# CederGroupHub/sparse-lm

Hardware: AMD Instinct MI355X
Metric: fits/sec over 50-alpha Lasso path at n=100k p=5k (higher is better)
Workload: dtype f64

## Files before the change

sparse-lm_amd/csrc/host_logic.hpp:

```cpp
#pragma once
#include <stddef.h>
#include <math.h>
#include <stdint.h>
#include <stdio.h>
#include <stdlib.h>

#include <algorithm>
#include <utility>
#include <vector>

#if defined(__HIPCC__)
#define SLM_HD __host__ __device__
#else
#define SLM_HD
#endif

namespace slm_host {

struct PoolLedger {
  struct Idle { int dev; size_t bytes; void* block; };
  struct Live { void* block; int dev; size_t bytes; };
  std::vector<Idle> idle;
  std::vector<Live> live;
  size_t idle_bytes = 0;

  void* take(int dev, size_t bytes) {
    for (size_t i = 0; i < idle.size(); ++i) {
      if (idle[i].dev == dev && idle[i].bytes == bytes) {
        void* p = idle[i].block;
        idle.erase(idle.begin() + (long)i);
        idle_bytes -= bytes;
        live.push_back({p, dev, bytes});
        return p;
      }
    }
    return nullptr;
  }
  void adopt(void* p, int dev, size_t bytes) { live.push_back({p, dev, bytes}); }

  bool give_back(void* p, size_t cap, bool pooling, std::vector<void*>* evict) {
    for (size_t i = 0; i < live.size(); ++i) {
      if (live[i].block != p) continue;
      const int dev = live[i].dev;
      const size_t bytes = live[i].bytes;
      live.erase(live.begin() + (long)i);
      if (!pooling || bytes > cap) return false;
      while (idle_bytes + bytes > cap && !idle.empty()) {
        evict->push_back(idle.front().block);
        idle_bytes -= idle.front().bytes;
        idle.erase(idle.begin());
      }
      idle.push_back({dev, bytes, p});
      idle_bytes += bytes;
      return true;
    }
    return false;
  }
  std::vector<void*> retire_device(int dev) {
    std::vector<void*> out;
    for (const Live& e : live)
      if (e.dev == dev) return out;
    for (size_t i = 0; i < idle.size();) {
      if (idle[i].dev == dev) {
        out.push_back(idle[i].block);
        idle_bytes -= idle[i].bytes;
        idle.erase(idle.begin() + (long)i);
      } else {
        ++i;
      }
    }
    return out;
  }
  std::vector<void*> flush() {
    std::vector<void*> out;
    for (const Idle& e : idle) out.push_back(e.block);
    idle.clear();
    idle_bytes = 0;
    return out;
  }
};

inline int row_sets(int n_lanes, const void* const* row_weight, const int64_t* n_eff, int* set_of, int* set_lane) {
  int n_sets = 0;
  for (int l = 0; l < n_lanes; ++l) {
    int found = -1;
    for (int m = 0; m < l && found < 0; ++m)
      if (row_weight[m] == row_weight[l] && n_eff[m] == n_eff[l]) found = set_of[m];
    if (found < 0) {
      found = n_sets;
      set_lane[n_sets++] = l;
    }
    set_of[l] = found;
  }
  return n_sets;
}

struct LaneWalk {
  int32_t first;
  int32_t n_points;
  int32_t stride;
  int32_t tail_pt;
};
inline LaneWalk interleaved_walk(int lane, int B, int64_t total, bool tail_band, bool slack_deep = false) {
  LaneWalk w;
  w.first = lane;
  w.n_points = (int32_t)total;
  w.stride = B;
  w.tail_pt = -1;
  const int64_t rem = total % B, n_reg = total - rem;
  if (slack_deep && tail_band && total > 2 * (int64_t)B && total <= 3 * (int64_t)B) {
    const int64_t e = (3 * (int64_t)B - total) / 2, F = B - e;
    if (e >= 1 && F >= 1) {
      if (lane >= F) {
        w.n_points = (int32_t)B;
      } else {
        w.n_points = (int32_t)(B + F);
        const int64_t t = B + F + lane;
        if (t < total) w.tail_pt = (int32_t)t;
      }
      return w;
    }
  }
  if (tail_band && rem > 0 && n_reg >= 2 * (int64_t)B) {
    w.n_points = (int32_t)n_reg;
    if (lane >= B - rem) w.tail_pt = (int32_t)(n_reg + (lane - (B - rem)));
  }
  return w;
}
inline int64_t interleaved_points(const LaneWalk& w) {
  const int64_t regular = w.n_points > w.first ? ((int64_t)w.n_points - w.first + w.stride - 1) / w.stride : 0;
  return regular + (w.tail_pt >= 0 ? 1 : 0);
}

struct XtrGrid { int xb, yb, rows; };
inline int auto_path_lanes(int64_t n_points, int cap, bool big, bool wide_ok) {
  if (n_points < 1) n_points = 1;
  const int narrow = (int)std::min<int64_t>(std::min(cap, 16), n_points);
  if (!big || cap < 20 || n_points <= 16) return narrow;
  int best = narrow;
  double best_cost = 1.45 * (double)((n_points + 15) / 16);
  auto offer = [&](int64_t lanes) {
    lanes = std::min(lanes, n_points);
    if (lanes <= 16 || lanes > cap) return;
    const int64_t passes = (n_points + lanes - 1) / lanes;
    const double cost = (double)passes * ((lanes <= 20 ? 1.03 : 1.22) + 0.45);
    if (cost < best_cost - 1e-9) {
      best_cost = cost;
      best = (int)lanes;
    }
  };
  offer(18);
  offer(20);
  if (wide_ok)
    for (int64_t passes = 1; passes <= (n_points + 20) / 21; ++passes) {
      const int64_t lanes = (n_points + passes - 1) / passes;
      if (lanes > 20 && lanes <= 32) offer(lanes);
    }
  return best;
}

inline int xtr_row_blocks_most(int cus, int64_t ld, int col_block) {
  const int xb = (int)((ld + col_block - 1) / col_block);
  return std::max(1, 2 * cus / xb);
}
inline XtrGrid xtr_grid(int64_t n, int64_t ld, int col_block, int64_t want) {
  XtrGrid g;
  g.xb = (int)((ld + col_block - 1) / col_block);
  if (want < 1) want = 1;
  int64_t rows = (n + want - 1) / want;
  rows = (rows + 7) / 8 * 8;
  g.rows = (int)rows;
  g.yb = (int)((n + rows - 1) / rows);
  return g;
}

constexpr int kSampleThreads = 256;
constexpr int kSampleWgsPerCu = 4;
constexpr int kSampleMinRows = 16;
struct SamplePlan {
  int xb, yb;
  int64_t rows;
  int64_t ld32;
};
inline int64_t sample_ld32(int64_t p) { return (p + 3) / 4 * 4; }
inline SamplePlan sample_plan(int64_t n_s, int64_t p, int64_t ld32, int cus) {
  SamplePlan g;
  g.ld32 = ld32;
  (void)p;
  const int64_t quads = ld32 / 4;
  g.xb = (int)std::max<int64_t>(1, (quads + kSampleThreads - 1) / kSampleThreads);
  if (n_s < 1) n_s = 1;
  const int64_t want = std::max<int64_t>(1, (int64_t)kSampleWgsPerCu * std::max(1, cus) / g.xb);
  g.rows = std::max<int64_t>(kSampleMinRows, (n_s + want - 1) / want);
  g.yb = (int)((n_s + g.rows - 1) / g.rows);
  return g;
}

template <typename Entry>
inline int find_by_fingerprint(const std::vector<Entry>& entries, double fp1, double fp2, double n_eff) {
  for (size_t i = 0; i < entries.size(); ++i)
    if (entries[i].fp1 == fp1 && entries[i].fp2 == fp2 && entries[i].n_eff == n_eff) return (int)i;
  return -1;
}

inline void triangle_tile(int t, int* I_out, int* J_out) {
  int I = 0;
  while ((I + 1) * (I + 2) / 2 <= t) ++I;
  *I_out = I;
  *J_out = t - I * (I + 1) / 2;
}
inline int triangle_tiles(int side) { return side * (side + 1) / 2; }
SLM_HD inline void triangle_tile_fast(int t, int* I_out, int* J_out) {
  int I = (int)((sqrtf(8.0f * (float)t + 1.0f) - 1.0f) * 0.5f);
  while (I * (I + 1) / 2 > t) --I;
  while ((I + 1) * (I + 2) / 2 <= t) ++I;
  *I_out = I;
  *J_out = t - I * (I + 1) / 2;
}

inline int model_gram_cap(int64_t ld, double budget_bytes, int most) {
  const double each = 4.0 * (double)ld * (double)ld;
  return (int)std::max<double>(1.0, std::min<double>((double)most, budget_bytes / each));
}

constexpr int kSketchPowerIters = 1;
constexpr int kSketchRowDiv = 32;
constexpr int kWsLookahead = 2;
constexpr int kWsPowerIters = 10;

struct Knobs {
  bool split = true;
  double xtr_wgs_per_cu = 1.0;
  int grad_ring = -1;
  int grad_cfg[3] = {0, 0, 0};
  int rowdot_ring = -1;
  bool resid_vec = false;
  int cov_tile = 0;
  int power_iters = 0;
  int ws = -1;
  bool on_chip = true;
  int auto_lanes = 0;
  bool interleave = true;
  bool tail_band = true;
  bool carry = true;
  bool ws_carry = true;
  bool eval_fused = false;
  double ws_theta = 0.85;
  int ws_append = 48;
  int ws_kinit = 0;
  int ws_bb = 1;
  int ws_one_solver = 0;
  bool hard_callwide = false;
  int ws_miss_factor = 4;
  int ws_miss_div = 8;
  double ws_fill = 0.0;
  bool sample_start = true;
  int64_t sample_min_rows = 65536;
  int sample_div = 4;
  bool sample_f64 = false;
  int mg = -1;
  bool handover = true;
  bool light_pass = true;
  bool lag_handover = true;
  bool gram_owner = true;
  double device_pool_gb = -1.0;
  bool allow_any_arch = false;
  int trace = 0;
  bool trace_poll = false;

  template <typename Get>
  static Knobs from(Get get) {
    Knobs k;
    auto text = [&](const char* name) -> const char* { return get(name); };
    auto is_set = [&](const char* name) { return text(name) != nullptr; };
    auto first = [&](const char* name) -> char { const char* e = text(name); return e ? e[0] : '\0'; };
    auto as_int = [&](const char* name, int lo, int hi, int* out) {
      if (const char* e = text(name)) *out = std::max(lo, std::min(hi, atoi(e)));
    };
    k.split = first("SLM_SPLIT") != '0';
    if (const char* e = text("SLM_XTR_WGS_PER_CU")) {
      const double f = atof(e);
      if (f > 0.0 && f <= 2.0) k.xtr_wgs_per_cu = f;
    }
    if (const char c = first("SLM_GRAD_RING")) k.grad_ring = c == '0' ? 0 : (c == '1' ? 1 : -1);
    if (const char* e = text("SLM_GRAD_CONFIG")) {
      int W = 0, C = 0, R = 0;
      if (sscanf(e, "%d,%d,%d", &W, &C, &R) == 3) { k.grad_cfg[0] = W; k.grad_cfg[1] = C; k.grad_cfg[2] = R; }
    }
    if (const char c = first("SLM_ROWDOT_RING")) k.rowdot_ring = c == '1' ? 1 : 0;
    k.resid_vec = first("SLM_RESID_VEC") == '1';
    if (const char* e = text("SLM_COV_TILE")) k.cov_tile = atoi(e);
    if (const char* e = text("SLM_POWER_ITERS")) k.power_iters = std::max(2, atoi(e));
    if (const char c = first("SLM_WS")) k.ws = c == '0' ? 0 : (c == '1' ? 1 : -1);
    k.on_chip = first("SLM_ON_CHIP") != '0';
    if (const char* e = text("SLM_AUTO_LANES")) k.auto_lanes = std::max(1, atoi(e));
    k.interleave = !is_set("SLM_NO_INTERLEAVE");
    k.tail_band = !is_set("SLM_NO_TAIL_BAND");
    k.carry = !is_set("SLM_NO_CARRY");
    k.ws_carry = !is_set("SLM_NO_WS_CARRY");
    k.eval_fused = is_set("SLM_EVAL_FUSED");
    if (const char* e = text("SLM_WS_THETA")) {
      const double v = atof(e);
      if (v > 0.0 && v <= 1.0) k.ws_theta = v;
    }
    as_int("SLM_WS_APPEND", 1, 512, &k.ws_append);
    as_int("SLM_WS_KINIT", 16, 512, &k.ws_kinit);
    if (const char* e = text("SLM_WS_BB")) k.ws_bb = atoi(e) != 0;
    if (const char* e = text("SLM_WS_ONE_SOLVER")) k.ws_one_solver = atoi(e) != 0;
    k.hard_callwide = is_set("SLM_HARD_CALLWIDE");
    as_int("SLM_WS_MISS_FACTOR", 1, 8, &k.ws_miss_factor);
    as_int("SLM_WS_MISS_DIV", 1, 4096, &k.ws_miss_div);
    if (const char* e = text("SLM_WS_FILL")) k.ws_fill = std::max(0.1, std::min(1.0, atof(e)));
    k.sample_start = !is_set("SLM_NO_SAMPLE_START");
    if (const char* e = text("SLM_SAMPLE_START_MIN_ROWS")) k.sample_min_rows = std::max<int64_t>(64, atoll(e));
    as_int("SLM_SAMPLE_DIV", 1, 64, &k.sample_div);
    k.sample_f64 = first("SLM_SAMPLE_F64") == '1';
    if (const char c = first("SLM_MG")) k.mg = c == '0' ? 0 : (c == '2' ? 2 : -1);
    k.handover = !is_set("SLM_NO_HANDOVER");
    k.light_pass = !is_set("SLM_NO_LIGHT_PASS");
    k.gram_owner = !is_set("SLM_NO_GRAM_OWNER");
    k.lag_handover = !is_set("SLM_NO_LAG_HANDOVER");
    if (const char* e = text("SLM_DEVICE_POOL_GB")) k.device_pool_gb = std::max(0.0, atof(e));
    k.allow_any_arch = is_set("SLM_ALLOW_ANY_ARCH");
    if (const char c = first("SLM_TRACE")) k.trace = (c >= '1' && c <= '3') ? c - '0' : 1;
    k.trace_poll = is_set("SLM_TRACE_POLL");
    return k;
  }
};

}
```

sparse-lm_amd/csrc/ws_kernels.hpp:

```cpp
#pragma once
#include <type_traits>
#include <hip/hip_runtime.h>
#include <stdint.h>

#include "tail_kernels.hpp"
#include "newton_kernels.hpp"

namespace slm {

constexpr int WS_KCAP = 512;
constexpr int WS_KLDS = 112;
constexpr int WS_TILES = WS_KCAP / 16;
constexpr int WS_THREADS = 1024;
constexpr int WS_INNER_MAX = 400;
constexpr int WS_BB_ITERS = 14;
constexpr double WS_BB_MAX_STEP = 20.0;
constexpr double WS_INNER_TOL = 0.05;
constexpr int WS_MAX_REPEATS = 6;
constexpr int WS_NEWTON_AFTER = 16;
constexpr int WS_NEWTON_MAX = 256;
constexpr int WS_AFTER_DIRECT = 40;
constexpr double WS_NEWTON_RQ = 0.05;
constexpr int WS_NEWTON_REFUSALS = 4;
constexpr double WS_NEWTON_ENTER = 0.3;
constexpr int WS_NEWTON_RESOLVE = 5;
static_assert(NT_MAXT * NT_B == WS_KCAP, "the direct solve covers a full working set");

struct WsCtl {
  int32_t request;
  int32_t building;
  int32_t valid;
  int32_t K;
  int32_t Kreal;
  int32_t k_new;
  int32_t builds;
  int32_t appends;
  int32_t max_builds;
  int32_t disabled;
  int32_t misses;
  int32_t refined;
  int32_t counter;
  int32_t stale;
  int32_t overflows;
  int32_t sweep_new;
  int32_t sweep_miss;
  int32_t staged;
  int32_t inner_iters;
  int32_t hard;
  int32_t hard_next;
  int32_t newton_steps;
  int32_t newton_fails;
  int32_t newton_nopd;
  int32_t newton_trial[4];
  int32_t newton_ref[4];
  int32_t newton_factors;
  int32_t newton_unknowns;
  unsigned long long nt_ticks[SLM_MAX_LANES][6];
  int32_t nt_factors[SLM_MAX_LANES];
  unsigned long long solve_ticks[5];
  int32_t want_full[SLM_MAX_LANES];
  int32_t iters_hist[32];
  unsigned long long lane_ticks[SLM_MAX_LANES];
  int32_t last_point[SLM_MAX_LANES];
  int32_t repeats[SLM_MAX_LANES];
  int32_t last_cols[SLM_MAX_LANES];
  double Lw[SLM_MAX_LANES];
  int32_t carried;
  int32_t outgrown;
  int32_t served[SLM_MAX_LANES];
  int32_t hard_lane[SLM_MAX_LANES];
};

struct WsArgs {
  WsCtl* ws;
  int32_t* idx;
  int32_t* pos;
  int32_t* gs;
  int32_t* gl;
  double* score;
  double* XW;
  double* part;
  double* Gm;
  double* nt;
  double* Gx;
  const double* X;
  const double* XT;
  int64_t n, ld;
  const double* rw;
  int64_t rw_stride;
  double inv_n[SLM_MAX_LANES];
  int32_t set_of[SLM_MAX_LANES];
  int32_t set_lane[SLM_MAX_LANES];
  int32_t n_sets;
  int32_t nblk;
  const int32_t* owner;
  double theta;
  int32_t lookahead;
  int32_t append_max;
  int32_t k_init;
  int32_t bb_steps;
  int32_t one_solver;
  int32_t miss_factor;
  int32_t miss_div;
  double fill;
  int32_t power_iters;
  int32_t hard_call;
  int32_t keep_full;
};

constexpr int WS_HEAD_WORDS = 24;
static_assert(offsetof(WsCtl, hard_next) / 4 < WS_HEAD_WORDS, "the words the pass kernels decide on");
#define WS_HEAD(hd, field) ((hd)[offsetof(WsCtl, field) / 4])
__device__ __forceinline__ void ws_head_load(const WsCtl* ws, const int* gdone, int32_t* hd) {
  const int tid = threadIdx.x;
  if (tid < WS_HEAD_WORDS) hd[tid] = reinterpret_cast<const int32_t*>(ws)[tid];
  else if (tid == WS_HEAD_WORDS) hd[tid] = gdone ? gdone[0] : 0;
}

static __global__ void ws_ctl_init_kernel(WsCtl* ws, int max_builds) {
  if (threadIdx.x == 0) {
    ws->request = 1;
    ws->max_builds = max_builds;
  }
  if (threadIdx.x < SLM_MAX_LANES) ws->last_point[threadIdx.x] = -1;
}

struct BeginArgs {
  const PathCtl* h_ctl;
  PathCtl* ctl;
  const slm_path_point* h_pts;
  slm_path_point* pts;
  int64_t n_pts;
  int32_t* head;
  int32_t head_words;
  const double* lambda;
  double margin;
  double factor[SLM_MAX_LANES];
  WsCtl* ws;
  int32_t max_builds;
  int32_t n_lanes;
};
static __global__ __launch_bounds__(256) void solve_begin_kernel(SetupArgs s, BeginArgs b) {
  solve_setup_body(s);
  const int64_t stride = (int64_t)gridDim.x * blockDim.x;
  {
    static_assert(sizeof(slm_path_point) == 4 * sizeof(double), "points travel as doubles");
    const double* src = reinterpret_cast<const double*>(b.h_pts);
    double* dst = reinterpret_cast<double*>(b.pts);
    for (int64_t e = (int64_t)blockIdx.x * blockDim.x + threadIdx.x; e < 4 * b.n_pts; e += stride) dst[e] = src[e];
  }
  if (blockIdx.x != 0) return;
  for (int e = threadIdx.x; e < b.head_words; e += 256) b.head[e] = 0;
  {
    static_assert(sizeof(PathCtl) % sizeof(int32_t) == 0, "control blocks travel as words");
    const int32_t* src = reinterpret_cast<const int32_t*>(b.h_ctl);
    int32_t* dst = reinterpret_cast<int32_t*>(b.ctl);
    const int words = b.n_lanes * (int)(sizeof(PathCtl) / sizeof(int32_t));
    for (int e = threadIdx.x; e < words; e += 256) dst[e] = src[e];
  }
  __syncthreads();
  if (b.lambda != nullptr && (int)threadIdx.x < b.n_lanes && threadIdx.x < SLM_MAX_LANES) {
    const int l = threadIdx.x;
    double L0 = b.lambda[0] * b.margin;
    if (L0 <= 0.0) L0 = 1.0;
    const double L = L0 * b.factor[l];
    b.ctl[l].L = L;
    b.ctl[l].ak = 1.25 * L;
    b.ctl[l].Lhat = 0.5 * L0;
  }
  if (b.ws != nullptr) {
    if (threadIdx.x == 0) {
      b.ws->request = 1;
      b.ws->max_builds = b.max_builds;
    }
    if (threadIdx.x < SLM_MAX_LANES) b.ws->last_point[threadIdx.x] = -1;
  }
}

static __global__ __launch_bounds__(256) void ws_ctl_carry_kernel(WsCtl* ws, int max_builds) {
  __shared__ int keep_i[2];
  __shared__ double keep_L[SLM_MAX_LANES];
  if (threadIdx.x == 0) {
    keep_i[0] = ws->K;
    keep_i[1] = ws->Kreal;
  }
  if (threadIdx.x < SLM_MAX_LANES) keep_L[threadIdx.x] = ws->Lw[threadIdx.x];
  __syncthreads();
  int32_t* words = reinterpret_cast<int32_t*>(ws);
  for (int e = threadIdx.x; e < (int)(sizeof(WsCtl) / sizeof(int32_t)); e += 256) words[e] = 0;
  __syncthreads();
  if (threadIdx.x == 0) {
    ws->K = keep_i[0];
    ws->Kreal = keep_i[1];
    ws->valid = 1;
    ws->carried = 1;
    ws->max_builds = max_builds;
  }
  if (threadIdx.x < SLM_MAX_LANES) {
    ws->Lw[threadIdx.x] = keep_L[threadIdx.x];
    ws->last_point[threadIdx.x] = -1;
  }
}

__device__ __forceinline__ int block_excl_scan(int v, int* wave_tot , int* total) {
  const int lane = threadIdx.x & 63, wave = threadIdx.x >> 6;
  int inc = v;
#pragma unroll
  for (int off = 1; off < 64; off <<= 1) {
    const int t = __shfl_up(inc, off, 64);
    if (lane >= off) inc += t;
  }
  __syncthreads();
  if (lane == 63) wave_tot[wave] = inc;
  __syncthreads();
  int base = 0, tot = 0;
#pragma unroll
  for (int w = 0; w < TAIL_WAVES; ++w) {
    const int t = wave_tot[w];
    if (w < wave) base += t;
    tot += t;
  }
  *total = tot;
  return base + inc - v;
}

__device__ __forceinline__ void ws_score_body(TailArgs a, WsArgs w, const int chunk) {
  WsCtl* ws = w.ws;
  const int tid = threadIdx.x;
  __shared__ int32_t hd[WS_HEAD_WORDS + 1];
  __shared__ int lane_np[SLM_MAX_LANES];
  ws_head_load(ws, a.gdone, hd);
  if (tid < SLM_MAX_LANES) lane_np[tid] = tid < a.n_lanes ? a.ctl[tid].n_points : 0;
  __syncthreads();
  if (hd[WS_HEAD_WORDS] != 0 || WS_HEAD(hd, disabled)) return;
  const bool had_w = WS_HEAD(hd, valid) != 0;
  if (!WS_HEAD(hd, request) && !had_w) return;
  if (WS_HEAD(hd, builds) >= WS_HEAD(hd, max_builds) || WS_HEAD(hd, appends) >= 8 * WS_HEAD(hd, max_builds)) return;
  const bool singleton = a.singleton != 0;
  const int nitems = singleton ? a.p : a.G;
  __shared__ int lane_live[SLM_MAX_LANES];
  __shared__ double lane_sa[SLM_MAX_LANES], lane_sb[SLM_MAX_LANES];
  __shared__ int cnt[2];
  if (tid < SLM_MAX_LANES) {
    int live = 0;
    double sa = 0.0, sb = 0.0;
    if (tid < a.n_lanes) {
      const PathCtl* c = a.ctl + tid;
      live = !(c->done || c->idle);
      int path_end = 0;
      for (int l = 0; l < SLM_MAX_LANES; ++l) path_end = max(path_end, lane_np[l]);
      const int end = a.steal ? path_end : c->pt_off + c->n_points;
      int look = min(c->pt_off + c->point + max(w.lookahead, c->stride), end - 1);
      if (c->tail_pt >= 0 && c->point + c->stride >= c->n_points) look = c->pt_off + c->tail_pt;
      const slm_path_point pe = a.pts[look < 0 ? 0 : look];
      sa = pe.sa;
      sb = pe.sb;
    }
    lane_live[tid] = live;
    lane_sa[tid] = sa;
    lane_sb[tid] = sb;
  }
  if (tid == 0) cnt[0] = cnt[1] = 0;
  __syncthreads();

  const double inf = __builtin_huge_val();
  int n_new = 0, n_miss = 0;
  const int gt = chunk * (int)blockDim.x + tid;
  const int it = singleton ? gt : gt >> 4;
  if (singleton) {
    if (it < nitems) {
      double sc = 0.0;
      const int j = it;
      const bool in_w = had_w && w.pos[j] >= 0;
      for (int l0 = 0; l0 < a.n_lanes; l0 += 16) {
        double zp[16], zz[16], aa[16], bb[16], gg[16];
#pragma unroll
        for (int l = 0; l < 16; ++l) {
          const int ll = l0 + l < a.n_lanes ? l0 + l : 0;
          const int64_t off = (int64_t)ll * a.ld;
          zp[l] = a.zprev[off + j];
          zz[l] = a.z[off + j];
          aa[l] = a.a0[off + j];
          bb[l] = a.b0[off + j];
          gg[l] = a.g[(int64_t)ll * (a.ld + 16) + j];
        }
#pragma unroll
        for (int l = 0; l < 16; ++l) {
          if (l0 + l >= a.n_lanes || !lane_live[l0 + l]) continue;
          if (!in_w && had_w && zz[l] != zp[l]) n_miss += 1;
          if (zp[l] != 0.0) {
            sc = inf;
          } else {
            const double thr = lane_sa[l0 + l] * aa[l] + lane_sb[l0 + l] * bb[l];
            sc = fmax(sc, thr > 0.0 ? fabs(gg[l]) / thr : inf);
          }
        }
      }
      if (sc >= w.theta && !in_w) n_new += 1;
      w.score[it] = sc;
    }
  } else {
    static_assert(SLM_MAX_LANES % 16 == 0, "16-thread teams: a thread per (group, lane of a half)");
    const int l16 = tid & 15;
    const bool have = it < nitems;
    double sc = 0.0;
    bool in_w = false;
    int k0 = 0, k1 = 0;
    if (have) {
      k0 = a.gstart[it];
      k1 = a.gstart[it + 1];
      in_w = had_w && w.pos[a.order[k0]] >= 0;
    }
    for (int l = l16; have && l < a.n_lanes; l += 16) {
      if (lane_live[l]) {
        const int64_t off = (int64_t)l * a.ld;
        const double* g = a.g + (int64_t)l * (a.ld + 16);
        double num = 0.0, rmax = 0.0;
        bool act = false;
        for (int k = k0; k < k1; ++k) {
          const int j = a.order[k];
          const double zp = a.zprev[off + j], zj = a.z[off + j], aj = a.a0[off + j], gj = g[j];
          if (!in_w && had_w && zj != zp) n_miss += 1;
          act = act || zp != 0.0;
          const double thr = lane_sa[l] * aj;
          const double m = fmax(fabs(gj) - thr, 0.0);
          num = __builtin_fma(m, m, num);
          rmax = fmax(rmax, thr > 0.0 ? fabs(gj) / thr : inf);
        }
        const double den = lane_sb[l] * a.b0[off + it];
        const double r = den > 0.0 ? sqrt(num) / den : rmax;
        sc = fmax(sc, act ? inf : r);
      }
    }
#pragma unroll
    for (int o = 8; o >= 1; o >>= 1) sc = fmax(sc, __shfl_xor(sc, o, 64));
    if (have && l16 == 0) {
      if (sc >= w.theta && !in_w) n_new += k1 - k0;
      w.score[it] = sc;
    }
  }
  if (n_new) atomicAdd(&cnt[0], n_new);
  if (n_miss) atomicAdd(&cnt[1], n_miss);
  __syncthreads();
  if (tid == 0) {
    if (cnt[0]) atomicAdd(&ws->sweep_new, cnt[0]);
    if (cnt[1]) atomicAdd(&ws->sweep_miss, cnt[1]);
  }
}

static __global__ __launch_bounds__(256) void ws_score_kernel(TailArgs a, WsArgs w) { ws_score_body(a, w, (int)blockIdx.x); }

__device__ __forceinline__ void ws_select_body(TailArgs a, WsArgs w) {
  __shared__ double red[2][TAIL_WAVES];
  __shared__ int wave_tot[TAIL_WAVES];
  WsCtl* ws = w.ws;
  if (threadIdx.x < SLM_MAX_LANES) ws->served[threadIdx.x] = 0;
  if (a.gdone[0] != 0 || ws->disabled) return;
  const int tid = threadIdx.x;
  const int p = a.p, G = a.G;
  const bool singleton = a.singleton != 0;
  const int nitems = singleton ? p : G;
  const bool had_w = ws->valid != 0;

  if (tid == 0 && ws->hard_next) ws->hard = 1;
  const bool requested = ws->request != 0;
  if (!requested && !had_w) return;
  if (ws->builds >= ws->max_builds || ws->appends >= 8 * ws->max_builds) {
    if (tid == 0) {
      ws->request = 0;
      ws->stale = 1;
    }
    return;
  }

  double sweep[2] = {(double)ws->sweep_new, (double)ws->sweep_miss};
  const bool carried = ws->carried != 0;
  __syncthreads();
  if (tid == 0) {
    ws->sweep_new = 0;
    ws->sweep_miss = 0;
    ws->carried = 0;
  }
  const double inf = __builtin_huge_val();
  const bool miss = had_w && sweep[1] != 0.0;
  if (miss && tid == 0) ws->misses += 1;
  if (had_w && !requested && sweep[0] == 0.0) {
    if (miss && tid == 0) ws->stale = 1;
    return;
  }

  const int per = (nitems + WS_THREADS - 1) / WS_THREADS;
  const int i0 = tid * per, i1 = min(i0 + per, nitems);
  const bool cached = per <= 8;
  double c_sc[8];
  int c_sz[8];
  bool c_inw[8];
  if (cached) {
    int first[8];
#pragma unroll
    for (int u = 0; u < 8; ++u) {
      const int it = (i0 + u < i1) ? i0 + u : 0;
      c_sc[u] = (i0 + u < i1) ? w.score[it] : -1.0;
      first[u] = singleton ? it : a.gstart[it];
      c_sz[u] = singleton ? 1 : a.gstart[it + 1] - first[u];
    }
    if (!singleton) {
#pragma unroll
      for (int u = 0; u < 8; ++u) first[u] = a.order[first[u]];
    }
#pragma unroll
    for (int u = 0; u < 8; ++u) c_inw[u] = w.pos[first[u]] >= 0;
  }

  auto count_at = [&](double thr, bool only_new, double* n_sel, double* smax) {
    double v[2] = {0.0, 0.0};
    if (cached) {
#pragma unroll
      for (int u = 0; u < 8; ++u) {
        if (c_sc[u] >= thr && !(only_new && c_inw[u])) v[0] += (double)c_sz[u];
        if (c_sc[u] < inf) v[1] = fmax(v[1], c_sc[u]);
      }
    } else {
      for (int it = tid; it < nitems; it += WS_THREADS) {
        const double sc = w.score[it];
        const int first = singleton ? it : a.order[a.gstart[it]];
        const int size = singleton ? 1 : a.gstart[it + 1] - a.gstart[it];
        if (sc >= thr && !(only_new && w.pos[first] >= 0)) v[0] += (double)size;
        if (sc < inf) v[1] = fmax(v[1], sc);
      }
    }
    double s[1] = {v[0]};
    block_sum<1>(s, red);
    *n_sel = s[0];
    if (smax == nullptr) return;
    double m = v[1];
#pragma unroll
    for (int off = 32; off >= 1; off >>= 1) m = fmax(m, __shfl_xor(m, off, 64));
    __syncthreads();
    if ((tid & 63) == 0) red[1][tid >> 6] = m;
    __syncthreads();
    double mm = 0.0;
#pragma unroll
    for (int k = 0; k < TAIL_WAVES; ++k) mm = fmax(mm, red[1][k]);
    *smax = mm;
  };

  auto fit_threshold = [&](double thr0, bool only_new, double cap, double* n_out) -> double {
    double n_sel, smax;
    count_at(thr0, only_new, &n_sel, &smax);
    if (n_sel <= cap) {
      *n_out = n_sel;
      return thr0;
    }
    double lo = thr0, hi = fmax(smax, thr0) * (1.0 + 1e-12) + 1e-300;
    double n_hi = 0.0;
    for (int k = 0; k < 14; ++k) {
      const double mid = 0.5 * (lo + hi);
      count_at(mid, only_new, &n_sel, nullptr);
      if (n_sel > cap) {
        lo = mid;
      } else {
        hi = mid;
        n_hi = n_sel;
        if (n_sel >= w.fill * cap) break;
      }
    }
    if (n_hi == 0.0) count_at(hi, only_new, &n_hi, nullptr);
    *n_out = n_hi;
    return hi;
  };

  double n_sel, smax, thr = w.theta;
  const int k_old = had_w ? ws->Kreal : 0;
  bool append = had_w;
  if (append) {
    const int miss_mult = miss ? min(w.miss_factor, 1 + (int)sweep[1] / max(w.miss_div, 1)) : 1;
    const double cap = (double)(carried ? max(w.k_init, 4 * w.append_max) : miss_mult * w.append_max);
    if (sweep[0] <= cap) {
      n_sel = sweep[0];
    } else {
      thr = fit_threshold(w.theta, true, cap, &n_sel);
    }
    if (n_sel == 0.0) {
      if (tid == 0) ws->request = 0;
      return;
    }
    if ((double)k_old + n_sel > (double)WS_KCAP) {
      if (tid == 0) ws->outgrown += 1;
      if (w.keep_full) {
        double nz_now;
        count_at(inf, false, &nz_now, nullptr);
        if (nz_now > 0.75 * (double)WS_KCAP) {
          if (tid == 0) {
            ws->request = 0;
            ws->stale = 1;
          }
          return;
        }
      }
      append = false;
      thr = w.theta;
    }
  }
  if (!append) {
    count_at(inf, false, &n_sel, nullptr);
    if (n_sel > (double)WS_KCAP) {
      if (tid == 0) {
        ws->overflows += 1;
        ws->outgrown += 1;
        if (had_w) {
          ws->request = 0;
          ws->stale = 1;
        } else {
          ws->request = 1;
          ws->valid = 0;
          if (ws->overflows >= 50) ws->disabled = 1;
        }
      }
      return;
    }
    const double nonzeros = n_sel;
    thr = fit_threshold(w.theta, false, fmax((double)w.k_init, nonzeros), &n_sel);
    for (int j = tid; j < p; j += WS_THREADS) w.pos[j] = -1;
  }
  for (int k = k_old * (append ? 1 : 0) + tid; k < WS_KCAP; k += WS_THREADS) {
    w.idx[k] = -1;
    w.gs[k] = k;
    w.gl[k] = 1;
  }
  __syncthreads();

  unsigned long long pick = 0ull;
  int mine = 0;
  if (cached) {
#pragma unroll
    for (int u = 0; u < 8; ++u) {
      if (c_sc[u] >= thr && !(append && c_inw[u])) {
        pick |= 1ull << u;
        mine += c_sz[u];
      }
    }
  } else {
    for (int it = i0; it < i1 && it - i0 < 64; ++it) {
      if (!(w.score[it] >= thr)) continue;
      if (append && w.pos[singleton ? it : a.order[a.gstart[it]]] >= 0) continue;
      pick |= 1ull << (it - i0);
      mine += singleton ? 1 : a.gstart[it + 1] - a.gstart[it];
    }
  }
  int total = 0;
  int at = (append ? k_old : 0) + block_excl_scan(mine, wave_tot, &total);
  __syncthreads();
  for (int it = i0; it < i1 && it - i0 < 64; ++it) {
    if (!((pick >> (it - i0)) & 1ull)) continue;
    if (singleton) {
      w.idx[at] = it;
      w.pos[it] = at;
      at += 1;
    } else {
      const int k0 = a.gstart[it], len = a.gstart[it + 1] - k0;
      for (int m = 0; m < len; ++m) {
        const int j = a.order[k0 + m];
        w.idx[at + m] = j;
        w.pos[j] = at + m;
        w.gs[at + m] = at;
        w.gl[at + m] = len;
      }
      at += len;
    }
  }
  if (tid == 0) {
    const int Kreal = (append ? k_old : 0) + total;
    ws->Kreal = Kreal;
    ws->K = max(16, (Kreal + 15) & ~15);
    ws->k_new = append ? k_old : 0;
    ws->building = 1;
    ws->valid = 0;
    ws->stale = 0;
    ws->counter = 0;
    if (append) {
      ws->appends += 1;
    } else {
      ws->builds += 1;
      for (int l = 0; l < SLM_MAX_LANES; ++l) ws->Lw[l] = 0.0;
    }
  }
}

static __global__ __launch_bounds__(WS_THREADS) void ws_select_kernel(TailArgs a, WsArgs w) { ws_select_body(a, w); }

static __global__ __launch_bounds__(256) void ws_gather_kernel(WsArgs w) {
  if (!w.ws->building) return;
  const int K = w.ws->K;
  const int k0 = w.ws->k_new + 32 * (int)blockIdx.y;
  if (k0 >= K) return;
  __shared__ double tile[32][33];
  const int tx = threadIdx.x & 31, ty = threadIdx.x >> 5;
  const int64_t row_tiles = (w.n + 31) / 32;
  int jcol[4];
#pragma unroll
  for (int u = 0; u < 4; ++u) {
    const int k = k0 + ty + 8 * u;
    jcol[u] = k < K ? w.idx[k] : -1;
  }
  for (int64_t rt = blockIdx.x; rt < row_tiles; rt += gridDim.x) {
    const int64_t i0 = rt * 32;
    const int64_t i = i0 + tx;
    double v[4];
#pragma unroll
    for (int u = 0; u < 4; ++u) {
      const int j = jcol[u];
      v[u] = (j >= 0 && i < w.n) ? (w.XT ? w.XT[((rt * w.ld + j) << 5) + tx] : w.X[i * w.ld + j]) : 0.0;
    }
    __syncthreads();
#pragma unroll
    for (int u = 0; u < 4; ++u) tile[ty + 8 * u][tx] = v[u];
    __syncthreads();
    for (int ii = ty; ii < 32; ii += 8) {
      const int64_t i = i0 + ii;
      const int k = k0 + tx;
      if (i < w.n && k < K) w.XW[i * WS_KCAP + k] = tile[tx][ii];
    }
  }
}

struct XtyArgs {
  const WsCtl* ws;
  const int32_t* idx;
  const double* XW;
  const double* y;
  double* part;
  double* g;
  double* gprev;
  double* z;
  PathCtl* ctl;
  const int* done;
  int64_t n, ld;
  double inv_n;
  int n_lanes, nblk;
};
static __global__ __launch_bounds__(512) void ws_xty_partial_kernel(XtyArgs a) {
  if (*a.done) return;
  __shared__ double red[8][WS_KCAP];
  __shared__ double red_yy[8];
  const int K = a.ws->K;
  const int lane = threadIdx.x & 63, wave = threadIdx.x >> 6;
  const int64_t rows = (a.n + gridDim.x - 1) / gridDim.x;
  const int64_t i0 = (int64_t)blockIdx.x * rows, i1 = i0 + rows < a.n ? i0 + rows : a.n;
  double acc[WS_KCAP / 64];
#pragma unroll
  for (int c = 0; c < WS_KCAP / 64; ++c) acc[c] = 0.0;
  double yy = 0.0;
  auto rows4 = [&](auto NC) {
    constexpr int C = decltype(NC)::value;
    for (int64_t i = i0 + wave; i < i1; i += 32) {
      double xv[4][C], yv[4];
#pragma unroll
      for (int r = 0; r < 4; ++r) {
        const bool in = i + 8 * r < i1;
        const int64_t ii = in ? i + 8 * r : i;
        yv[r] = in ? a.y[ii] : 0.0;
#pragma unroll
        for (int c = 0; c < C; ++c) {
          const int k = lane + 64 * c;
          xv[r][c] = a.XW[ii * WS_KCAP + (k < K ? k : 64 * c)];
        }
      }
#pragma unroll
      for (int r = 0; r < 4; ++r) {
        yy = __builtin_fma(yv[r], yv[r], yy);
#pragma unroll
        for (int c = 0; c < C; ++c) acc[c] = __builtin_fma(lane + 64 * c < K ? xv[r][c] : 0.0, yv[r], acc[c]);
      }
    }
  };
  switch ((K + 63) >> 6) {
    case 1: rows4(std::integral_constant<int, 1>{}); break;
    case 2: rows4(std::integral_constant<int, 2>{}); break;
    case 3: rows4(std::integral_constant<int, 3>{}); break;
    case 4: rows4(std::integral_constant<int, 4>{}); break;
    case 5: rows4(std::integral_constant<int, 5>{}); break;
    case 6: rows4(std::integral_constant<int, 6>{}); break;
    case 7: rows4(std::integral_constant<int, 7>{}); break;
    default: rows4(std::integral_constant<int, 8>{}); break;
  }
  static_assert(WS_KCAP / 64 == 8, "eight chunks of 64 positions");
#pragma unroll
  for (int c = 0; c < WS_KCAP / 64; ++c) red[wave][lane + 64 * c] = acc[c];
  if (lane == 0) red_yy[wave] = yy;
  __syncthreads();
  double* out = a.part + (int64_t)blockIdx.x * (WS_KCAP + 1);
  const int k = threadIdx.x;
  if (k < K) {
    double sum = 0.0;
#pragma unroll
    for (int w = 0; w < 8; ++w) sum += red[w][k];
    out[k] = sum;
  }
  if (k == WS_KCAP - 1) {
    double sum = 0.0;
#pragma unroll
    for (int w = 0; w < 8; ++w) sum += red_yy[w];
    out[WS_KCAP] = sum;
  }
}
static __global__ __launch_bounds__(512) void ws_xty_apply_kernel(XtyArgs a) {
  if (*a.done) return;
  __shared__ double red[4][128];
  __shared__ double ry[512];
  const int K = a.ws->K;
  const int kl = threadIdx.x & 127, q = threadIdx.x >> 7;
  const int k = (int)blockIdx.x * 128 + kl;
  if ((int)blockIdx.x * 128 >= K) return;
  double s[8] = {0, 0, 0, 0, 0, 0, 0, 0};
  if (k < K) {
    int b = q;
    for (; b + 28 < a.nblk; b += 32) {
#pragma unroll
      for (int u = 0; u < 8; ++u) s[u] += a.part[(int64_t)(b + 4 * u) * (WS_KCAP + 1) + k];
    }
    for (; b < a.nblk; b += 4) s[0] += a.part[(int64_t)b * (WS_KCAP + 1) + k];
  }
  red[q][kl] = ((s[0] + s[1]) + (s[2] + s[3])) + ((s[4] + s[5]) + (s[6] + s[7]));
  if (blockIdx.x == 0) ry[threadIdx.x] = (int)threadIdx.x < a.nblk ? a.part[(int64_t)threadIdx.x * (WS_KCAP + 1) + WS_KCAP] : 0.0;
  __syncthreads();
  if (q == 0 && k < K) {
    const int j = a.idx[k];
    if (j >= 0) {
      const double c = -((red[0][kl] + red[1][kl]) + (red[2][kl] + red[3][kl])) * a.inv_n;
      for (int l = 0; l < a.n_lanes; ++l) {
        a.g[(int64_t)l * (a.ld + 16) + j] = c;
        a.gprev[(int64_t)l * a.ld + j] = c;
        a.z[(int64_t)l * a.ld + j] = 0.0;
      }
    }
  }
  if (blockIdx.x == 0) {
    for (int off = 256; off >= 1; off >>= 1) {
      if ((int)threadIdx.x < off) ry[threadIdx.x] += ry[threadIdx.x + off];
      __syncthreads();
    }
    if (threadIdx.x < (unsigned)a.n_lanes) {
      const int l = threadIdx.x;
      const double loss0 = 0.5 * ry[0] * a.inv_n;
      a.g[(int64_t)l * (a.ld + 16) + a.ld] = loss0;
      a.ctl[l].hist[0] = loss0;
      a.ctl[l].loss_base = loss0;
    }
  }
}

static __global__ __launch_bounds__(256) void ws_block_owner_kernel(const double* rw, int64_t rw_stride, WsArgs w, int32_t* owner) {
  __shared__ int cls[SLM_MAX_LANES];
  __shared__ int red[2][4];
  const int tid = threadIdx.x;
  const int64_t b = blockIdx.x;
  const int64_t base = w.n / w.nblk, rem = w.n % w.nblk;
  const int64_t r0 = b * base + (b < rem ? b : rem);
  const int64_t nrows = base + (b < rem ? 1 : 0);
  for (int st = 0; st < w.n_sets; ++st) {
    const double* v = rw + (int64_t)w.set_lane[st] * rw_stride + r0;
    int zeros = 1, ones = 1;
    for (int64_t i = tid; i < nrows; i += 256) {
      const double x = v[i];
      zeros &= (x == 0.0);
      ones &= (x == 1.0);
    }
    zeros = __all(zeros);
    ones = __all(ones);
    if ((tid & 63) == 0) {
      red[0][tid >> 6] = zeros;
      red[1][tid >> 6] = ones;
    }
    __syncthreads();
    if (tid == 0) {
      const int z = red[0][0] & red[0][1] & red[0][2] & red[0][3], o = red[1][0] & red[1][1] & red[1][2] & red[1][3];
      cls[st] = z ? 0 : (o ? 1 : 2);
    }
    __syncthreads();
  }
  if (tid == 0) {
    int first_ones = -1;
    for (int st = 0; st < w.n_sets; ++st) {
      int o = st;
      if (cls[st] == 0) o = -1;
      else if (cls[st] == 1) {
        if (first_ones < 0) first_ones = st;
        o = first_ones;
      }
      owner[(int64_t)st * w.nblk + b] = o;
    }
  }
}

typedef double ws_d4 __attribute__((ext_vector_type(4)));
constexpr int WS_GRAM_THREADS = 512;
constexpr int WS_GRAM_ZCHUNKS = 4;

static __global__ __launch_bounds__(WS_GRAM_THREADS) void ws_gram_kernel(WsArgs w) {
  if (!w.ws->building) return;
  __shared__ ws_d4 comb[2][16][64];
  const int K = w.ws->K;
  const int tile_lo = w.ws->k_new >> 4;
  const int tid = threadIdx.x, lane = tid & 63;
  const int wave = __builtin_amdgcn_readfirstlane(tid >> 6);
  const int tiles = K >> 4;
  const bool row_split = (tile_lo > 0 || tiles <= 8) && tiles - tile_lo <= 4 * WS_GRAM_ZCHUNKS;
  const int set = blockIdx.y;
  const int64_t b = blockIdx.x;
  if (w.owner != nullptr && w.owner[(int64_t)set * w.nblk + b] != set) return;
  const int64_t base = w.n / w.nblk, rem = w.n % w.nblk;
  const int64_t r0 = b * base + (b < rem ? b : rem);
  const int64_t nrows = base + (b < rem ? 1 : 0);
  const double* rw = w.rw ? w.rw + (int64_t)w.set_lane[set] * w.rw_stride : nullptr;
  const int part = row_split ? (wave >> 1) : 0;
  const int64_t steps = (nrows + 3) >> 2;
  const int64_t s_begin = row_split ? 4 * (steps * part / 4) : 0;
  const int64_t s_end = row_split ? min(nrows, 4 * (steps * (part + 1) / 4)) : nrows;

  for (int slice = 0; slice < 4 * WS_GRAM_ZCHUNKS; ++slice) {
  const int zhi = slice >> 2;
  if (8 * (slice & 3) >= tiles) continue;
  if (row_split ? (tile_lo + 4 * zhi >= tiles) : (zhi >= 2)) continue;
  const int wj = 2 * (slice & 3) + (wave & 1);
  const int ntj = min(4, max(0, tiles - 4 * wj));
  const int ibase = row_split ? tile_lo + 4 * zhi : 4 * (4 * zhi + (wave >> 1));
  const int ti_lo = row_split ? 0 : max(0, tile_lo - ibase);
  const int nti = min(4, max(0, tiles - ibase));
  const bool active = ti_lo < nti && ntj > 0;
  if (!row_split && !active) continue;
  ws_d4 acc[4][4];
#pragma unroll
  for (int ti = 0; ti < 4; ++ti)
#pragma unroll
    for (int tj = 0; tj < 4; ++tj) acc[ti][tj] = ws_d4{0.0, 0.0, 0.0, 0.0};

  const int kk = lane >> 4, c = lane & 15;
  if (active) {
    const int ta_max = WS_TILES - 1;
    const double* rwp = rw ? rw : w.XW;
    const bool has_rw = rw != nullptr;
    auto load = [&](int64_t s, double(&av)[4], double(&bv)[4], double& wgt) {
      const int64_t i = s + kk;
      const bool ok = i < s_end;
      const int64_t row = r0 + (ok ? i : 0);
      const double wv = rwp[has_rw ? row : 0];
      const double* xr = w.XW + row * WS_KCAP + c;
#pragma unroll
      for (int t = 0; t < 4; ++t) {
        av[t] = xr[16 * min(ibase + t, ta_max)];
        bv[t] = xr[16 * min(4 * wj + t, ta_max)];
      }
      wgt = ok ? (has_rw ? wv : 1.0) : 0.0;
    };
    auto mma = [&](const double(&av)[4], const double(&bv)[4], double wgt) {
#pragma unroll
      for (int ti = 0; ti < 4; ++ti) {
        if (ti >= ti_lo && ti < nti) {
          const double a = av[ti] * wgt;
#pragma unroll
          for (int tj = 0; tj < 4; ++tj)
            if (tj < ntj) acc[ti][tj] = __builtin_amdgcn_mfma_f64_16x16x4f64(a, bv[tj], acc[ti][tj], 0, 0, 0);
        }
      }
    };
    double a0[4], b0[4], a1[4], b1[4], a2[4], b2[4], a3[4], b3[4], w0, w1, w2, w3;
    load(s_begin, a0, b0, w0);
    load(s_begin + 4, a1, b1, w1);
    load(s_begin + 8, a2, b2, w2);
    for (int64_t s = s_begin; s < s_end; s += 16) {
      load(s + 12, a3, b3, w3);
      mma(a0, b0, w0);
      load(s + 16, a0, b0, w0);
      mma(a1, b1, w1);
      load(s + 20, a1, b1, w1);
      mma(a2, b2, w2);
      load(s + 24, a2, b2, w2);
      mma(a3, b3, w3);
    }
  }
  if (row_split) {
    for (int round = 0; round < 4; ++round) {
      if (part == round && active) {
#pragma unroll
        for (int ti = 0; ti < 4; ++ti)
#pragma unroll
          for (int tj = 0; tj < 4; ++tj) {
            if (ti < nti && tj < ntj) {
              if (round > 0) acc[ti][tj] += comb[wave & 1][ti * 4 + tj][lane];
              if (round < 3) comb[wave & 1][ti * 4 + tj][lane] = acc[ti][tj];
            }
          }
      }
      __syncthreads();
    }
  }
  if (!row_split || (part == 3 && active)) {
#pragma unroll
  for (int ti = 0; ti < 4; ++ti) {
    if (ti < ti_lo || ti >= nti) continue;
#pragma unroll
    for (int tj = 0; tj < 4; ++tj) {
      if (tj >= ntj) continue;
      const int64_t tile = (int64_t)(ibase + ti) * WS_TILES + (4 * wj + tj);
      double* out = w.part + (((int64_t)set * (WS_TILES * WS_TILES) + tile) * w.nblk + b) * 256;
#pragma unroll
      for (int r = 0; r < 4; ++r) out[(kk + 4 * r) * 16 + c] = acc[ti][tj][r];
    }
  }
  }
  if (row_split) __syncthreads();
  }
}

static __global__ __launch_bounds__(256) void ws_gram_reduce_kernel(WsArgs w) {
  WsCtl* ws = w.ws;
  if (!ws->building) return;
  const int K = ws->K;
  const int row_lo = (ws->k_new >> 4) << 4;
  const int set = blockIdx.y;
  const int tile = blockIdx.x, I = tile / WS_TILES, J = tile % WS_TILES;
  const int tiles = K >> 4, I_lo = row_lo >> 4;
  if (I < I_lo || I >= tiles || J >= tiles) return;
  const int i = 16 * I + (threadIdx.x >> 4), j = 16 * J + (threadIdx.x & 15);
  {
    const double* src = w.part + (((int64_t)set * (WS_TILES * WS_TILES) + tile) * w.nblk) * 256 + threadIdx.x;
    double s4[4] = {0.0, 0.0, 0.0, 0.0};
    int b = 0;
    if (w.owner != nullptr) {
      __shared__ int64_t off_s[512];
      static_assert(sizeof(off_s) >= 8 * 512, "nblk <= 512");
      for (int bb = threadIdx.x; bb < w.nblk; bb += 256) {
        const int o = w.owner[(int64_t)set * w.nblk + bb];
        off_s[bb] = o < 0 ? -1 : (int64_t)(o - set) * (WS_TILES * WS_TILES) * w.nblk * 256;
      }
      __syncthreads();
      for (; b + 32 <= w.nblk; b += 32) {
        double v[32];
#pragma unroll
        for (int u = 0; u < 32; ++u) {
          const int64_t o = off_s[b + u];
          v[u] = o == -1 ? 0.0 : src[(int64_t)(b + u) * 256 + o];
        }
#pragma unroll
        for (int u = 0; u < 32; ++u) s4[u & 3] += v[u];
      }
      for (; b < w.nblk; ++b) {
        const int64_t o = off_s[b];
        s4[b & 3] += o == -1 ? 0.0 : src[(int64_t)b * 256 + o];
      }
    }
    for (; b + 32 <= w.nblk; b += 32) {
      double v[32];
#pragma unroll
      for (int u = 0; u < 32; ++u) v[u] = src[(int64_t)(b + u) * 256];
#pragma unroll
      for (int u = 0; u < 32; ++u) s4[u & 3] += v[u];
    }
    for (; b < w.nblk; ++b) s4[b & 3] += src[(int64_t)b * 256];
    double s = ((s4[0] + s4[1]) + (s4[2] + s4[3])) * w.inv_n[set];
    double* Gs = (w.Gx ? w.Gx : w.Gm) + (int64_t)set * (WS_KCAP * WS_KCAP);
    Gs[i * WS_KCAP + j] = s;
    if (j < row_lo) Gs[j * WS_KCAP + i] = s;
  }
  __threadfence();
  __syncthreads();
  if (threadIdx.x == 0) {
    const int total = (tiles - I_lo) * tiles * (int)gridDim.y;
    if (atomicAdd(&ws->counter, 1) + 1 == total) {
      ws->counter = 0;
      if (w.Gx) {
        ws->staged = 1;
      } else {
        ws->request = 0;
        ws->valid = 1;
        __threadfence();
        ws->building = 0;
      }
    }
  }
}

constexpr int WS_PUBLISH_BLOCKS = 64;
static __global__ __launch_bounds__(256) void ws_publish_kernel(WsArgs w) {
  WsCtl* ws = w.ws;
  if (!ws->building || !ws->staged) return;
  const int K = ws->K;
  const int row_lo = (ws->k_new >> 4) << 4;
  const int set = blockIdx.y;
  for (int i = blockIdx.x; i < K; i += gridDim.x)
    for (int j = threadIdx.x; j < K; j += 256)
      if (i >= row_lo || j >= row_lo) {
        const int64_t at = (int64_t)set * (WS_KCAP * WS_KCAP) + (int64_t)i * WS_KCAP + j;
        w.Gm[at] = w.Gx[at];
      }
  __threadfence();
  __syncthreads();
  if (threadIdx.x == 0) {
    const int total = gridDim.x * gridDim.y;
    if (atomicAdd(&ws->counter, 1) + 1 == total) {
      ws->counter = 0;
      ws->staged = 0;
      ws->request = 0;
      ws->valid = 1;
      __threadfence();
      ws->building = 0;
    }
  }
}

constexpr int SSE_M = 16;

struct GatherArgs {
  const double* X;
  const double* XT;
  int64_t n, ld;
  const int32_t* idx;
  int K;
  double* XW;
};

static __global__ __launch_bounds__(256) void gather_cols_kernel(GatherArgs w) {
  const int k0 = 32 * (int)blockIdx.y;
  if (k0 >= w.K) return;
  __shared__ double tile[32][33];
  const int tx = threadIdx.x & 31, ty = threadIdx.x >> 5;
  const int64_t row_tiles = (w.n + 31) / 32;
  for (int64_t rt = blockIdx.x; rt < row_tiles; rt += gridDim.x) {
    const int64_t i0 = rt * 32;
    __syncthreads();
    for (int kk = ty; kk < 32; kk += 8) {
      const int k = k0 + kk;
      const int j = k < w.K ? w.idx[k] : -1;
      const int64_t i = i0 + tx;
      tile[kk][tx] = (j >= 0 && i < w.n) ? (w.XT ? w.XT[((rt * w.ld + j) << 5) + tx] : w.X[i * w.ld + j]) : 0.0;
    }
    __syncthreads();
    for (int ii = ty; ii < 32; ii += 8) {
      const int64_t i = i0 + ii;
      const int k = k0 + tx;
      if (i < w.n && k < w.K) w.XW[i * WS_KCAP + k] = tile[tx][ii];
    }
  }
}

struct SseArgs {
  const double* XW;
  const double* y;
  const double* rw;
  const double* Zs;
  double* partial;
  int64_t n;
  int K, m;
};

static __global__ __launch_bounds__(256) void sse_sparse_kernel(SseArgs a) {
  extern __shared__ double zs[];
  __shared__ double wsum[4][SSE_M];
  const int tid = threadIdx.x, lane = tid & 63, wave = tid >> 6;
  for (int e = tid; e < a.K * SSE_M; e += 256) {
    const int k = e / SSE_M, v = e - k * SSE_M;
    zs[e] = v < a.m ? a.Zs[(int64_t)v * a.K + k] : 0.0;
  }
  __syncthreads();
  double sse[SSE_M];
#pragma unroll
  for (int v = 0; v < SSE_M; ++v) sse[v] = 0.0;
  for (int64_t row = (int64_t)blockIdx.x * 256 + tid; row < a.n; row += (int64_t)gridDim.x * 256) {
    const double w = a.rw ? a.rw[row] : 1.0;
    if (w == 0.0) continue;
    const double* xr = a.XW + row * WS_KCAP;
    double dot[SSE_M];
#pragma unroll
    for (int v = 0; v < SSE_M; ++v) dot[v] = 0.0;
    for (int k = 0; k < a.K; ++k) {
      const double x = xr[k];
#pragma unroll
      for (int v = 0; v < SSE_M; ++v) dot[v] = __builtin_fma(x, zs[k * SSE_M + v], dot[v]);
    }
    const double yi = a.y[row];
#pragma unroll
    for (int v = 0; v < SSE_M; ++v) {
      const double e = dot[v] - yi;
      sse[v] = __builtin_fma(w * e, e, sse[v]);
    }
  }
#pragma unroll
  for (int v = 0; v < SSE_M; ++v) {
    double t = sse[v];
#pragma unroll
    for (int off = 32; off >= 1; off >>= 1) t += __shfl_xor(t, off, 64);
    if (lane == 0) wsum[wave][v] = t;
  }
  __syncthreads();
  if (tid < SSE_M) a.partial[(int64_t)blockIdx.x * SSE_M + tid] = wsum[0][tid] + wsum[1][tid] + wsum[2][tid] + wsum[3][tid];
}

}
```

Before: 17480.

## Compute only lower-triangle Gram tiles in row-split working-set build

The row-split Gram path now assigns each wave a set of tiles restricted to the lower triangle (J<=I). Columns are strided by two across the wave pair, and a per-tile mask skips the upper-triangle MFMAs and their partial-sum writes. The load/MFMA loop is templated on tile counts so the compiler drops unused loads and branches. The reduce kernel skips upper-triangle tiles and mirrors the results, with its completion counter adjusted to match. This roughly halves the MFMA work for the Gram update, but adds a 16-way dispatch switch and more complex tile bookkeeping that the completion counter depends on.

```diff
diff --git a/sparse-lm_amd/csrc/host_logic.hpp b/sparse-lm_amd/csrc/host_logic.hpp
--- a/sparse-lm_amd/csrc/host_logic.hpp
+++ b/sparse-lm_amd/csrc/host_logic.hpp
@@ -216,6 +216,51 @@
   while ((I + 1) * (I + 2) / 2 <= t) ++I;
   *I_out = I;
   *J_out = t - I * (I + 1) / 2;
+}
+
+constexpr int kGramChunks = 4;
+constexpr int kGramPasses = 4;
+struct GramDeal {
+  int ibase, nti;
+  int col0, ntj;
+  unsigned mask;
+};
+SLM_HD inline bool gram_row_split(int tile_lo, int tiles) {
+  return (tile_lo > 0 || tiles <= 8) && tiles - tile_lo <= 4 * kGramChunks;
+}
+SLM_HD inline void gram_row_quarter(int64_t nrows, int part, int64_t* begin, int64_t* end) {
+  const int64_t steps = (nrows + 3) >> 2;
+  const int64_t e = 4 * (steps * (part + 1) / 4);
+  *begin = 4 * (steps * part / 4);
+  *end = e < nrows ? e : nrows;
+}
+SLM_HD inline bool gram_deal(int tile_lo, int tiles, int chunk, int pass, int h, GramDeal* d) {
+  const int nnew = tiles - tile_lo;
+  const int nch = (nnew + 3) >> 2;
+  if (chunk >= nch) return false;
+  const int rper = (nnew + nch - 1) / nch;
+  int ibase = tile_lo + rper * chunk;
+  if (ibase >= tiles) return false;
+  int nti = rper < tiles - ibase ? rper : tiles - ibase;
+  const int jmax = ibase + nti - 1;
+  if (8 * pass > jmax) return false;
+  const int col0 = 8 * pass + h;
+  int ntj = col0 > jmax ? 0 : (jmax - col0) / 2 + 1;
+  if (ntj > 4) ntj = 4;
+  if (col0 > ibase && ntj > 0) {
+    nti -= col0 - ibase;
+    ibase = col0;
+  }
+  unsigned mask = 0;
+  for (int ti = 0; ti < nti; ++ti)
+    for (int tj = 0; tj < ntj; ++tj)
+      if (col0 + 2 * tj <= ibase + ti) mask |= 1u << (4 * ti + tj);
+  d->ibase = ibase;
+  d->nti = nti;
+  d->col0 = col0;
+  d->ntj = ntj;
+  d->mask = mask;
+  return true;
 }
 
 inline int model_gram_cap(int64_t ld, double budget_bytes, int most) {
diff --git a/sparse-lm_amd/csrc/ws_kernels.hpp b/sparse-lm_amd/csrc/ws_kernels.hpp
--- a/sparse-lm_amd/csrc/ws_kernels.hpp
+++ b/sparse-lm_amd/csrc/ws_kernels.hpp
@@ -3,6 +3,7 @@
 #include <hip/hip_runtime.h>
 #include <stdint.h>
 
+#include "host_logic.hpp"
 #include "tail_kernels.hpp"
 #include "newton_kernels.hpp"
 
@@ -797,6 +798,46 @@
 constexpr int WS_GRAM_THREADS = 512;
 constexpr int WS_GRAM_ZCHUNKS = 4;
 
+template <int NTI, int NTJ>
+__device__ __forceinline__ void ws_gram_rows(const double* __restrict__ XW, const double* __restrict__ rwp, const bool has_rw,
+                                             const int64_t r0, const int64_t s_begin, const int64_t s_end, const int kk, const int c,
+                                             const int ibase, const int col0, const int cstep, ws_d4 (&acc)[4][4]) {
+  const int ta_max = WS_TILES - 1;
+  auto load = [&](int64_t s, double(&av)[NTI], double(&bv)[NTJ], double& wv) {
+    const int64_t i = s + kk;
+    const int64_t row = r0 + (i < s_end ? i : 0);
+    wv = rwp[has_rw ? row : 0];
+    const double* xr = XW + row * WS_KCAP + c;
+#pragma unroll
+    for (int t = 0; t < NTI; ++t) av[t] = xr[16 * min(ibase + t, ta_max)];
+#pragma unroll
+    for (int t = 0; t < NTJ; ++t) bv[t] = xr[16 * min(col0 + cstep * t, ta_max)];
+  };
+  auto mma = [&](int64_t s, const double(&av)[NTI], const double(&bv)[NTJ], double wv) {
+    const double wgt = s + kk < s_end ? (has_rw ? wv : 1.0) : 0.0;
+#pragma unroll
+    for (int ti = 0; ti < NTI; ++ti) {
+      const double a = av[ti] * wgt;
+#pragma unroll
+      for (int tj = 0; tj < NTJ; ++tj) acc[ti][tj] = __builtin_amdgcn_mfma_f64_16x16x4f64(a, bv[tj], acc[ti][tj], 0, 0, 0);
+    }
+  };
+  double a0[NTI], b0[NTJ], a1[NTI], b1[NTJ], a2[NTI], b2[NTJ], a3[NTI], b3[NTJ], w0, w1, w2, w3;
+  load(s_begin, a0, b0, w0);
+  load(s_begin + 4, a1, b1, w1);
+  load(s_begin + 8, a2, b2, w2);
+  for (int64_t s = s_begin; s < s_end; s += 16) {
+    load(s + 12, a3, b3, w3);
+    mma(s, a0, b0, w0);
+    load(s + 16, a0, b0, w0);
+    mma(s + 4, a1, b1, w1);
+    load(s + 20, a1, b1, w1);
+    mma(s + 8, a2, b2, w2);
+    load(s + 24, a2, b2, w2);
+    mma(s + 12, a3, b3, w3);
+  }
+}
+
 static __global__ __launch_bounds__(WS_GRAM_THREADS) void ws_gram_kernel(WsArgs w) {
   if (!w.ws->building) return;
   __shared__ ws_d4 comb[2][16][64];
@@ -805,7 +846,8 @@
   const int tid = threadIdx.x, lane = tid & 63;
   const int wave = __builtin_amdgcn_readfirstlane(tid >> 6);
   const int tiles = K >> 4;
-  const bool row_split = (tile_lo > 0 || tiles <= 8) && tiles - tile_lo <= 4 * WS_GRAM_ZCHUNKS;
+  const bool row_split = slm_host::gram_row_split(tile_lo, tiles);
+  static_assert(slm_host::kGramChunks == WS_GRAM_ZCHUNKS, "the slices of the row-split deal");
   const int set = blockIdx.y;
   const int64_t b = blockIdx.x;
   if (w.owner != nullptr && w.owner[(int64_t)set * w.nblk + b] != set) return;
@@ -814,20 +856,36 @@
   const int64_t nrows = base + (b < rem ? 1 : 0);
   const double* rw = w.rw ? w.rw + (int64_t)w.set_lane[set] * w.rw_stride : nullptr;
   const int part = row_split ? (wave >> 1) : 0;
-  const int64_t steps = (nrows + 3) >> 2;
-  const int64_t s_begin = row_split ? 4 * (steps * part / 4) : 0;
-  const int64_t s_end = row_split ? min(nrows, 4 * (steps * (part + 1) / 4)) : nrows;
+  int64_t s_begin = 0, s_end = nrows;
+  if (row_split) slm_host::gram_row_quarter(nrows, part, &s_begin, &s_end);
 
   for (int slice = 0; slice < 4 * WS_GRAM_ZCHUNKS; ++slice) {
   const int zhi = slice >> 2;
-  if (8 * (slice & 3) >= tiles) continue;
-  if (row_split ? (tile_lo + 4 * zhi >= tiles) : (zhi >= 2)) continue;
-  const int wj = 2 * (slice & 3) + (wave & 1);
-  const int ntj = min(4, max(0, tiles - 4 * wj));
-  const int ibase = row_split ? tile_lo + 4 * zhi : 4 * (4 * zhi + (wave >> 1));
-  const int ti_lo = row_split ? 0 : max(0, tile_lo - ibase);
-  const int nti = min(4, max(0, tiles - ibase));
-  const bool active = ti_lo < nti && ntj > 0;
+  int ibase, col0, cstep, nti, ntj;
+  unsigned msk = 0;
+  if (row_split) {
+    slm_host::GramDeal d;
+    if (!slm_host::gram_deal(tile_lo, tiles, zhi, slice & 3, wave & 1, &d)) continue;
+    ibase = d.ibase;
+    nti = d.nti;
+    col0 = d.col0;
+    ntj = d.ntj;
+    cstep = 2;
+    msk = d.mask;
+  } else {
+    if (8 * (slice & 3) >= tiles || zhi >= 2) continue;
+    const int wj = 2 * (slice & 3) + (wave & 1);
+    ntj = min(4, max(0, tiles - 4 * wj));
+    ibase = max(4 * (4 * zhi + (wave >> 1)), tile_lo);
+    nti = max(0, min(tiles, 4 * (4 * zhi + (wave >> 1)) + 4) - ibase);
+    col0 = 4 * wj;
+    cstep = 1;
+    for (int ti = 0; ti < nti; ++ti) msk |= ((1u << ntj) - 1u) << (4 * ti);
+  }
+  msk = __builtin_amdgcn_readfirstlane(msk);
+  nti = __builtin_amdgcn_readfirstlane(nti);
+  ntj = __builtin_amdgcn_readfirstlane(ntj);
+  const bool active = msk != 0;
   if (!row_split && !active) continue;
   ws_d4 acc[4][4];
 #pragma unroll
@@ -837,47 +895,17 @@
 
   const int kk = lane >> 4, c = lane & 15;
   if (active) {
-    const int ta_max = WS_TILES - 1;
     const double* rwp = rw ? rw : w.XW;
-    const bool has_rw = rw != nullptr;
-    auto load = [&](int64_t s, double(&av)[4], double(&bv)[4], double& wgt) {
-      const int64_t i = s + kk;
-      const bool ok = i < s_end;
-      const int64_t row = r0 + (ok ? i : 0);
-      const double wv = rwp[has_rw ? row : 0];
-      const double* xr = w.XW + row * WS_KCAP + c;
-#pragma unroll
-      for (int t = 0; t < 4; ++t) {
-        av[t] = xr[16 * min(ibase + t, ta_max)];
-        bv[t] = xr[16 * min(4 * wj + t, ta_max)];
-      }
-      wgt = ok ? (has_rw ? wv : 1.0) : 0.0;
-    };
-    auto mma = [&](const double(&av)[4], const double(&bv)[4], double wgt) {
-#pragma unroll
-      for (int ti = 0; ti < 4; ++ti) {
-        if (ti >= ti_lo && ti < nti) {
-          const double a = av[ti] * wgt;
-#pragma unroll
-          for (int tj = 0; tj < 4; ++tj)
-            if (tj < ntj) acc[ti][tj] = __builtin_amdgcn_mfma_f64_16x16x4f64(a, bv[tj], acc[ti][tj], 0, 0, 0);
-        }
-      }
-    };
-    double a0[4], b0[4], a1[4], b1[4], a2[4], b2[4], a3[4], b3[4], w0, w1, w2, w3;
-    load(s_begin, a0, b0, w0);
-    load(s_begin + 4, a1, b1, w1);
-    load(s_begin + 8, a2, b2, w2);
-    for (int64_t s = s_begin; s < s_end; s += 16) {
-      load(s + 12, a3, b3, w3);
-      mma(a0, b0, w0);
-      load(s + 16, a0, b0, w0);
-      mma(a1, b1, w1);
-      load(s + 20, a1, b1, w1);
-      mma(a2, b2, w2);
-      load(s + 24, a2, b2, w2);
-      mma(a3, b3, w3);
-    }
+#define WS_GRAM_CASE(I, J) \
+  case 4 * (I - 1) + (J - 1): ws_gram_rows<I, J>(w.XW, rwp, rw != nullptr, r0, s_begin, s_end, kk, c, ibase, col0, cstep, acc); break;
+    switch (4 * (nti - 1) + (ntj - 1)) {
+      WS_GRAM_CASE(1, 1) WS_GRAM_CASE(1, 2) WS_GRAM_CASE(1, 3) WS_GRAM_CASE(1, 4)
+      WS_GRAM_CASE(2, 1) WS_GRAM_CASE(2, 2) WS_GRAM_CASE(2, 3) WS_GRAM_CASE(2, 4)
+      WS_GRAM_CASE(3, 1) WS_GRAM_CASE(3, 2) WS_GRAM_CASE(3, 3) WS_GRAM_CASE(3, 4)
+      WS_GRAM_CASE(4, 1) WS_GRAM_CASE(4, 2) WS_GRAM_CASE(4, 3) WS_GRAM_CASE(4, 4)
+      default: break;
+    }
+#undef WS_GRAM_CASE
   }
   if (row_split) {
     for (int round = 0; round < 4; ++round) {
@@ -886,7 +914,7 @@
         for (int ti = 0; ti < 4; ++ti)
 #pragma unroll
           for (int tj = 0; tj < 4; ++tj) {
-            if (ti < nti && tj < ntj) {
+            if ((msk >> (4 * ti + tj)) & 1u) {
               if (round > 0) acc[ti][tj] += comb[wave & 1][ti * 4 + tj][lane];
               if (round < 3) comb[wave & 1][ti * 4 + tj][lane] = acc[ti][tj];
             }
@@ -898,11 +926,10 @@
   if (!row_split || (part == 3 && active)) {
 #pragma unroll
   for (int ti = 0; ti < 4; ++ti) {
-    if (ti < ti_lo || ti >= nti) continue;
 #pragma unroll
     for (int tj = 0; tj < 4; ++tj) {
-      if (tj >= ntj) continue;
-      const int64_t tile = (int64_t)(ibase + ti) * WS_TILES + (4 * wj + tj);
+      if (!((msk >> (4 * ti + tj)) & 1u)) continue;
+      const int64_t tile = (int64_t)(ibase + ti) * WS_TILES + (col0 + cstep * tj);
       double* out = w.part + (((int64_t)set * (WS_TILES * WS_TILES) + tile) * w.nblk + b) * 256;
 #pragma unroll
       for (int r = 0; r < 4; ++r) out[(kk + 4 * r) * 16 + c] = acc[ti][tj][r];
@@ -922,8 +949,10 @@
   const int tile = blockIdx.x, I = tile / WS_TILES, J = tile % WS_TILES;
   const int tiles = K >> 4, I_lo = row_lo >> 4;
   if (I < I_lo || I >= tiles || J >= tiles) return;
+  const bool tri = slm_host::gram_row_split(I_lo, tiles);
+  if (tri && J > I) return;
   const int i = 16 * I + (threadIdx.x >> 4), j = 16 * J + (threadIdx.x & 15);
-  {
+  if (J <= I) {
     const double* src = w.part + (((int64_t)set * (WS_TILES * WS_TILES) + tile) * w.nblk) * 256 + threadIdx.x;
     double s4[4] = {0.0, 0.0, 0.0, 0.0};
     int b = 0;
@@ -960,13 +989,15 @@
     for (; b < w.nblk; ++b) s4[b & 3] += src[(int64_t)b * 256];
     double s = ((s4[0] + s4[1]) + (s4[2] + s4[3])) * w.inv_n[set];
     double* Gs = (w.Gx ? w.Gx : w.Gm) + (int64_t)set * (WS_KCAP * WS_KCAP);
-    Gs[i * WS_KCAP + j] = s;
-    if (j < row_lo) Gs[j * WS_KCAP + i] = s;
+    if (j <= i) {
+      Gs[i * WS_KCAP + j] = s;
+      if (j < i) Gs[j * WS_KCAP + i] = s;
+    }
   }
   __threadfence();
   __syncthreads();
   if (threadIdx.x == 0) {
-    const int total = (tiles - I_lo) * tiles * (int)gridDim.y;
+    const int total = (tri ? (tiles * (tiles + 1) - I_lo * (I_lo + 1)) / 2 : (tiles - I_lo) * tiles) * (int)gridDim.y;
     if (atomicAdd(&ws->counter, 1) + 1 == total) {
       ws->counter = 0;
       if (w.Gx) {
```

Result: faster. 17670, median of 6 (+1.1%).
